# MohammadJohari/myslam

Measured on AMD Instinct MI355X. Metric: ray.samples/s (render+bwd), higher is better.
Workload: dtype f32; 1 GPU; BASELINE configs[1]: Replica room0 (synthetic), 4096 rays x 64 samples (56+8); mapping iteration: sample + render fwd + loss + bwd (planes+decoders), no optimiser; rays_of_the_job=4096, rays_this_rank=4096, samples_per_ray=64, plane_bytes=27147008, planes_layout=channels_last, parallelism=single GPU, launch=hipGraph replay of the captured iteration

## Files before the change

myslam_amd/csrc/eslam_decode_tile.h:

```cpp
#pragma once
#include "eslam_common.h"

__device__ __forceinline__ int piece_channel(int g, int i) { return i < 4 ? 4 * g + i : 12 + 4 * g + i; }

template <bool CL>
__device__ __forceinline__ void gather8(const eslam_plane_t& P, float u, float v, int q, float acc[8]) {
    const AxisCoord ax = axis_coord(u, P.w);
    const AxisCoord ay = axis_coord(v, P.h);
    const float w00 = (1.0f - ax.t) * (1.0f - ay.t);
    const float w01 = ax.t * (1.0f - ay.t);
    const float w10 = (1.0f - ax.t) * ay.t;
    const float w11 = ax.t * ay.t;
    const unsigned sy = (unsigned)P.stride_y, sx = (unsigned)P.stride_x;
    const unsigned r0 = ay.i0 * sy, r1 = ay.i1 * sy;
    const unsigned c0 = ax.i0 * sx, c1 = ax.i1 * sx;
    const float* __restrict__ data = P.data;
    if (CL) {
        const unsigned q4 = 4u * q;
        const unsigned o00 = r0 + c0 + q4, o01 = r0 + c1 + q4, o10 = r1 + c0 + q4, o11 = r1 + c1 + q4;
        const float4_t a00 = *(const float4_t*)(data + o00), b00 = *(const float4_t*)(data + o00 + 16u);
        const float4_t a01 = *(const float4_t*)(data + o01), b01 = *(const float4_t*)(data + o01 + 16u);
        const float4_t a10 = *(const float4_t*)(data + o10), b10 = *(const float4_t*)(data + o10 + 16u);
        const float4_t a11 = *(const float4_t*)(data + o11), b11 = *(const float4_t*)(data + o11 + 16u);
#pragma unroll
        for (int i = 0; i < 4; ++i) {
            acc[i] += a00[i] * w00 + a01[i] * w01 + a10[i] * w10 + a11[i] * w11;
            acc[4 + i] += b00[i] * w00 + b01[i] * w01 + b10[i] * w10 + b11[i] * w11;
        }
    } else {
        const unsigned sc = (unsigned)P.stride_c;
#pragma unroll
        for (int i = 0; i < 8; ++i) {
            const unsigned co = (unsigned)piece_channel(q, i) * sc;
            acc[i] += data[co + r0 + c0] * w00 + data[co + r0 + c1] * w01 + data[co + r1 + c0] * w10 +
                      data[co + r1 + c1] * w11;
        }
    }
}

struct DecFrag {
    float w1[16];
    float4_t w2;
    float4_t w3;
    float4_t b1, b2;
    float4_t b3;
};

__device__ __forceinline__ void load_dec_frag(DecFrag& f, const float* L, int r, int q) {
#pragma unroll
    for (int lvl = 0; lvl < 2; ++lvl) {
        const float4_t a = *(const float4_t*)(L + DEC_W1 + r * 64 + lvl * 32 + 4 * q);
        const float4_t b = *(const float4_t*)(L + DEC_W1 + r * 64 + lvl * 32 + 16 + 4 * q);
#pragma unroll
        for (int i = 0; i < 4; ++i) {
            f.w1[lvl * 8 + i] = a[i];
            f.w1[lvl * 8 + 4 + i] = b[i];
        }
    }
    f.w2 = *(const float4_t*)(L + DEC_W2 + r * 16 + 4 * q);
    f.w3 = *(const float4_t*)(L + DEC_W3 + (r & 3) * 16 + 4 * q);
    f.b1 = *(const float4_t*)(L + DEC_B1 + 4 * q);
    f.b2 = *(const float4_t*)(L + DEC_B2 + 4 * q);
    f.b3 = *(const float4_t*)(L + DEC_B3);
}

__device__ __forceinline__ void mlp_hidden2(const DecFrag& f, const float4_t& h1, float4_t& h2) {
    float4_t a2 = f.b2;
#pragma unroll
    for (int ks = 0; ks < 4; ++ks) a2 = mfma16(f.w2[ks], h1[ks], a2);
#pragma unroll
    for (int i = 0; i < 4; ++i) h2[i] = fmaxf(a2[i], 0.0f);
}

__device__ __forceinline__ void mlp_hidden(const DecFrag& f, const float feat[16], float4_t& h1, float4_t& h2) {
    float4_t a1 = f.b1;
#pragma unroll
    for (int ks = 0; ks < 16; ++ks) a1 = mfma16(f.w1[ks], feat[ks], a1);
#pragma unroll
    for (int i = 0; i < 4; ++i) h1[i] = fmaxf(a1[i], 0.0f);
    mlp_hidden2(f, h1, h2);
}

__device__ __forceinline__ int64_t hidden_blocks(int S) { return (S + 15) >> 4; }

__device__ __forceinline__ void mlp_out_accum(const DecFrag& f, const float4_t& h2, int b, int r, float4_t& out) {
    const bool mine = (r >> 2) == b;
#pragma unroll
    for (int ks = 0; ks < 4; ++ks) out = mfma16(mine ? f.w3[ks] : 0.0f, h2[ks], out);
}

#define GATHER_PIPELINE 1

struct PlaneTaps {
    float4_t a00, b00, a01, b01, a10, b10, a11, b11;
    float w00, w01, w10, w11;
};

__device__ __forceinline__ void issue_taps(const eslam_plane_t& P, float u, float v, int q, PlaneTaps& t) {
    const AxisCoord ax = axis_coord(u, P.w);
    const AxisCoord ay = axis_coord(v, P.h);
    t.w00 = (1.0f - ax.t) * (1.0f - ay.t);
    t.w01 = ax.t * (1.0f - ay.t);
    t.w10 = (1.0f - ax.t) * ay.t;
    t.w11 = ax.t * ay.t;
    const unsigned sy = (unsigned)P.stride_y, sx = (unsigned)P.stride_x;
    const unsigned r0 = ay.i0 * sy, r1 = ay.i1 * sy;
    const unsigned c0 = ax.i0 * sx, c1 = ax.i1 * sx;
    const float* __restrict__ data = P.data;
    const unsigned q4 = 4u * q;
    const unsigned o00 = r0 + c0 + q4, o01 = r0 + c1 + q4, o10 = r1 + c0 + q4, o11 = r1 + c1 + q4;
    t.a00 = *(const float4_t*)(data + o00); t.b00 = *(const float4_t*)(data + o00 + 16u);
    t.a01 = *(const float4_t*)(data + o01); t.b01 = *(const float4_t*)(data + o01 + 16u);
    t.a10 = *(const float4_t*)(data + o10); t.b10 = *(const float4_t*)(data + o10 + 16u);
    t.a11 = *(const float4_t*)(data + o11); t.b11 = *(const float4_t*)(data + o11 + 16u);
}

__device__ __forceinline__ void accumulate_taps(const PlaneTaps& t, float acc[8]) {
#pragma unroll
    for (int i = 0; i < 4; ++i) {
        acc[i] += t.a00[i] * t.w00 + t.a01[i] * t.w01 + t.a10[i] * t.w10 + t.a11[i] * t.w11;
        acc[4 + i] += t.b00[i] * t.w00 + t.b01[i] * t.w01 + t.b10[i] * t.w10 + t.b11[i] * t.w11;
    }
}

template <bool CL>
__device__ __forceinline__ void gather_features(const PlaneSet& planes, int d, float x, float y, float z, int q,
                                                float feat[16], int opaque0) {
#pragma unroll
    for (int i = 0; i < 16; ++i) feat[i] = 0.0f;
    if (CL && GATHER_PIPELINE) {
        constexpr int D = GATHER_PIPELINE + 1;
        PlaneTaps taps[D];
// ... 250 lines not shown
```

myslam_amd/csrc/eslam_mlp_bwd_dev.h:

```cpp
#pragma once
#include <type_traits>
#include "eslam_decode_tile.h"
#include "eslam_loss_final.h"

struct RayUp { float gd, gr, gg, gb; };

__device__ __forceinline__ float4_t composite_bwd_chunk(const RayUp up, float beta, bool valid, float sd, float z, float cr,
                                                        float cg, float cb, float g_sdf_s, float trans_in, float& carry,
                                                        float& gbeta_acc, int lane) {
    const float sg = sigmoidf_(-sd * beta);
    const float e = expf(-beta * sg);
    const float alpha = valid ? 1.0f - e : 0.0f;
    const float fac = valid ? (1.0f - alpha) + 1e-10f : 1.0f;
    const float pin = wave_incl_prod(fac, lane);
    const float pex = wave_up1(pin, 1.0f);
    const float T = trans_in * pex;
    const float w = alpha * T;
    const float gw = (up.gd != 0.0f ? up.gd * z : 0.0f) + up.gr * cr + up.gg * cg + up.gb * cb;
    const float v = valid ? gw * w : 0.0f;
    const float vn = wave_down1(v, 0.0f);
    const float after_local = wave_incl_suffix_sum(vn, lane);
    const float after = after_local + carry;
    const float g_alpha = gw * T - after / fac;
    carry += wave_lane<0>(after_local) + wave_lane<0>(v);
// ... 13 lines not shown
}

#define TP 20
#define TPF 68
#define TPH 72

struct RayBwdIn {
    const float* z_vals;
    const float* sdf;
    const float* raw_rgb;
    const float* beta;
    const float* g_depth;
    const float* g_rgb;
    const float* g_sdf;
    float* beta_parts;
    int R, S;
};

struct MlpBwdArgs {
    eslam_decoders_t dec;
    const float* feat;
    const float* g_o;
    int64_t N;
    float* g_feat;
    float* slabs;
    RayBwdIn rb;
    LossGradIn li;
    const float* hid;
};

struct MlpBwdLane {
    int d;
    int lane, wave;
    int r, q;
    int gp, gq;
};

__device__ __forceinline__ MlpBwdLane mlp_bwd_lane() {
    MlpBwdLane ln;
    ln.d = blockIdx.y;
    ln.lane = threadIdx.x & 63; ln.wave = threadIdx.x >> 6;
    ln.r = ln.lane & 15; ln.q = ln.lane >> 4;
    ln.gp = ln.lane >> 2; ln.gq = ln.lane & 3;
    return ln;
}

template <class T> __device__ __forceinline__ void mlp_bwd_touch(const T x) { asm volatile("" :: "v"(x)); }

struct MlpBwdLdsAll {
    __attribute__((aligned(16))) float wlds[2 * DEC_LDS];
    __attribute__((aligned(16))) float gtile[4][64 * 4];
};
template <bool LOWP> struct MlpBwdLdsWgrad {
    __attribute__((aligned(16))) float tiles[4][4][16 * TP];
    __attribute__((aligned(16))) float ftile[4][LOWP ? 16 * TPH / 2 : 16 * TPF];
    __attribute__((aligned(16))) float comb[4][SLAB];
};
struct MlpBwdLdsRays { float beta_part[4]; };
template <int> struct MlpBwdLdsNone {};
template <int MODE, bool WGRAD, bool LOWP>
struct MlpBwdLds : MlpBwdLdsAll, std::conditional_t<WGRAD, MlpBwdLdsWgrad<LOWP>, MlpBwdLdsNone<0>>,
                   std::conditional_t<MODE != 0, MlpBwdLdsRays, MlpBwdLdsNone<1>> {};

template <bool GZ> struct MlpBwdFragF32 {
    DecFrag f;
    float w3col[4], w2t[4], w1t[4][4];

    __device__ __forceinline__ void load(const float* wlds, const MlpBwdLane& ln) {
        const float* L = wlds + ln.d * DEC_LDS;
        const int r = ln.r, q = ln.q;
        load_dec_frag(f, L, r, q);
#pragma unroll
        for (int ks = 0; ks < 4; ++ks) {
            w3col[ks] = L[DEC_W3 + ks * 16 + r];
            w2t[ks] = L[DEC_W2 + (4 * q + ks) * 16 + r];
#pragma unroll
            for (int mb = 0; mb < 4; ++mb)
                if (!GZ) w1t[mb][ks] = L[DEC_W1 + (4 * q + ks) * 64 + (mb >> 1) * 32 + 16 * (mb & 1) + r];
        }
    }
};

struct MlpBwdFragBf16 {
    DecFragLP fl;
    short4_t w3colp = {0, 0, 0, 0}, w2tp = {0, 0, 0, 0}, w1tp[4];

    __device__ __forceinline__ void load(float* wlds, const MlpBwdLane& ln) {
        const int r = ln.r, q = ln.q;
        const short* W = lp_weights(wlds, ln.d);
        load_dec_frag_lp(fl, W, lp_biases(wlds, ln.d), r, q);
#pragma unroll
        for (int jj = 0; jj < 4; ++jj) {
            if (q == 0) w3colp[jj] = W[LP_W3 + jj * 16 + r];
            w2tp[jj] = W[LP_W2 + (4 * q + jj) * 16 + r];
#pragma unroll
            for (int mb = 0; mb < 4; ++mb) w1tp[mb][jj] = W[LP_W1 + (4 * q + jj) * 64 + 16 * mb + r];
        }
    }
};

template <bool LOWP, bool GZ> using MlpBwdFrag = std::conditional_t<LOWP, MlpBwdFragBf16, MlpBwdFragF32<GZ>>;

struct MlpBwdParamGrads {
    float4_t gW1[4], gW2, gW3, gb1, gb2;
    float gb3[3];

    __device__ __forceinline__ void clear() {
#pragma unroll
        for (int i = 0; i < 4; ++i) gW1[i] = (float4_t){0.f, 0.f, 0.f, 0.f};
        gW2 = gW3 = gb1 = gb2 = (float4_t){0.f, 0.f, 0.f, 0.f};
        gb3[0] = gb3[1] = gb3[2] = 0.f;
    }

    __device__ __forceinline__ void write_slab(float (*comb)[SLAB], float* __restrict__ slabs, const MlpBwdLane& ln) const {
        const int lane = ln.lane, r = ln.r, q = ln.q;
        const int nout = ln.d ? 3 : 1;
        float* sl = comb[ln.wave];
        for (int i = lane; i < SLAB; i += WAVE) sl[i] = 0.0f;
        WAVE_SYNC();
#pragma unroll
        for (int reg = 0; reg < 4; ++reg) {
            const int j = 4 * q + reg;
            float4_t v;
#pragma unroll
            for (int nb = 0; nb < 4; ++nb) v[nb] = gW1[nb][reg];
            *(float4_t*)(sl + SL_W1 + j * 64 + 4 * r) = v;
            sl[SL_W2 + j * 16 + r] = gW2[reg];
            if (q == 0 && reg < nout) sl[SL_W3 + reg * 16 + r] = gW3[reg];
        }
#pragma unroll
        for (int reg = 0; reg < 4; ++reg) {
            float a = gb1[reg], c = gb2[reg];
#pragma unroll
            for (int m = 8; m >= 1; m >>= 1) {
                a += __shfl_xor(a, m, WAVE);
                c += __shfl_xor(c, m, WAVE);
            }
            if (r == 0) {
                sl[SL_B1 + 4 * q + reg] = a;
                sl[SL_B2 + 4 * q + reg] = c;
            }
        }
#pragma unroll
        for (int o = 0; o < 3; ++o) {
            const float t = wave_sum(gb3[o]);
            if (lane == 0 && o < nout) sl[SL_B3 + o] = t;
        }
        __syncthreads();
        float* row = slabs + ((int64_t)blockIdx.x * 2 + ln.d) * SLAB;
        for (int col = threadIdx.x; col < SLAB; col += 256)
            row[col] = (comb[0][col] + comb[1][col]) + (comb[2][col] + comb[3][col]);
    }
};

template <bool GZ> struct MlpBwdGradOut {
    typedef unsigned uint4_t __attribute__((ext_vector_type(4)));
    __amdgpu_buffer_rsrc_t rsrc;
    unsigned gz_base;
    int d, gp, gq;

    __device__ __forceinline__ MlpBwdGradOut(float* g_feat, int64_t N, const MlpBwdLane& ln)
        : rsrc(__builtin_amdgcn_make_buffer_rsrc((void*)g_feat, 0, (int)((unsigned)N * (GZ ? 128u : 512u)), 0x00020000)),
          gz_base((unsigned)ln.d * ((unsigned)N * 64u)), d(ln.d), gp(ln.gp), gq(ln.gq) {}

    __device__ __forceinline__ void dropped_stores() const {
#pragma unroll
        for (int j = 0; j < (GZ ? 1 : 4); ++j) __builtin_amdgcn_raw_buffer_store_b128((uint4_t){0u, 0u, 0u, 0u}, rsrc, (int)(0xFFFFFF00u + 16u * j), 0, 0);
    }
    __device__ __forceinline__ void store_gz(const int64_t p0, const int b, const int nvalid, const float gzr[4]) const {
        const unsigned off = (16 * b + gp < nvalid) ? (unsigned)(p0 + 16 * b + gp) * 64u + gz_base + (unsigned)(gq * 16) : 0xFFFFFF00u;
        __builtin_amdgcn_raw_buffer_store_b128(__builtin_bit_cast(uint4_t, (float4_t){gzr[0], gzr[1], gzr[2], gzr[3]}), rsrc, (int)off, 0, 0);
    }
    __device__ __forceinline__ void store_rows(const int64_t p0, const int b, const int nvalid, const float gf[16]) const {
        const unsigned off = (16 * b + gp < nvalid) ? (unsigned)(p0 + 16 * b + gp) * 512u + (unsigned)(d * 256 + gq * 16) : 0xFFFFFF00u;
#pragma unroll
        for (int j = 0; j < 4; ++j)
            __builtin_amdgcn_raw_buffer_store_b128(__builtin_bit_cast(uint4_t, (float4_t){gf[4 * j], gf[4 * j + 1], gf[4 * j + 2], gf[4 * j + 3]}),
                                                   rsrc, (int)off + 64 * j, 0, 0);
    }
};

template <bool LOWP, bool ROWS, bool SAVEDH> struct MlpBwdPrefetch {
    float4_t fnext[4];
    float4_t hnext = (float4_t){0.f, 0.f, 0.f, 0.f};

    static __device__ __forceinline__ void load_block(const MlpBwdArgs& a, const MlpBwdLane& ln, float4_t v[4], const int64_t pbase) {
        const int64_t pt = min(pbase + ln.gp, a.N - 1);
        if (LOWP) {
            const short* fp = (const short*)a.feat + pt * 128 + ln.d * 64 + 8 * ln.gq;
            v[0] = *(const float4_t*)(fp);
            v[1] = *(const float4_t*)(fp + 32);
            v[2] = v[3] = (float4_t){0.f, 0.f, 0.f, 0.f};
            return;
        }
        const float* fp = a.feat + pt * 128 + ln.d * 64 + 4 * ln.gq;
        v[0] = *(const float4_t*)(fp);
        v[1] = *(const float4_t*)(fp + 16);
        v[2] = *(const float4_t*)(fp + 32);
        v[3] = *(const float4_t*)(fp + 48);
    }
    static __device__ __forceinline__ float4_t load_hidden(const MlpBwdArgs& a, const MlpBwdLane& ln, const int64_t hblk) {
        const int64_t hb_last = 2 * (int64_t)a.rb.R * hidden_blocks(a.rb.S) - 1;
        return *(const float4_t*)(a.hid + min(hblk, hb_last) * 256 + ln.lane * 4);
    }
    __device__ __forceinline__ void request(const MlpBwdArgs& a, const MlpBwdLane& ln, const int64_t pbase, const int64_t hblk) {
        if (ROWS) load_block(a, ln, fnext, pbase);
        if (SAVEDH) hnext = load_hidden(a, ln, hblk);
    }
    __device__ __forceinline__ void touch() const {
        if (ROWS) { mlp_bwd_touch(fnext[0]); mlp_bwd_touch(fnext[1]); mlp_bwd_touch(fnext[2]); mlp_bwd_touch(fnext[3]); }
        if (SAVEDH) mlp_bwd_touch(hnext);
    }
};

struct MlpBwdBlockOut { float4_t h1, h2, gz1, gz2; };

struct MlpBwdContract { float az1[4], az2[4], bh1[4], bh2[4], ago[4]; };
template <class Lds>
__device__ __forceinline__ MlpBwdContract mlp_bwd_transpose(Lds& lds, const MlpBwdLane& ln, const int b, const MlpBwdBlockOut& o) {
    const int r = ln.r, q = ln.q;
    float* tz1 = lds.tiles[ln.wave][0];
    float* tz2 = lds.tiles[ln.wave][1];
    float* th1 = lds.tiles[ln.wave][2];
    float* th2 = lds.tiles[ln.wave][3];
    const float* gt = lds.gtile[ln.wave];
    *(float4_t*)(tz1 + r * TP + 4 * q) = o.gz1;
    *(float4_t*)(tz2 + r * TP + 4 * q) = o.gz2;
    *(float4_t*)(th1 + r * TP + 4 * q) = o.h1;
    *(float4_t*)(th2 + r * TP + 4 * q) = o.h2;
    WAVE_SYNC();

    MlpBwdContract c;
#pragma unroll
    for (int ks = 0; ks < 4; ++ks) {
        const int prow = 4 * q + ks;
        c.az1[ks] = tz1[prow * TP + r];
        c.az2[ks] = tz2[prow * TP + r];
        c.bh1[ks] = th1[prow * TP + r];
        c.bh2[ks] = th2[prow * TP + r];
        c.ago[ks] = (r < 4) ? gt[(16 * b + prow) * 4 + r] : 0.0f;
    }
    return c;
}

__device__ __forceinline__ void mlp_bwd_stage_rows_f32(float* ftile, const MlpBwdLane& ln, const float ft[16]) {
    float* T = ftile + ln.gp * TPF + 4 * ln.gq;
#pragma unroll
    for (int j = 0; j < 4; ++j) *(float4_t*)(T + 16 * j) = (float4_t){ft[4 * j], ft[4 * j + 1], ft[4 * j + 2], ft[4 * j + 3]};
}

template <bool SAVEDH>
__device__ __forceinline__ void mlp_bwd_hidden_f32(const DecFrag& f, const float ft[16], const float4_t hsaved, float4_t& h1, float4_t& h2) {
    if (SAVEDH) { h1 = hsaved; mlp_hidden2(f, h1, h2); }
    else mlp_hidden(f, ft, h1, h2);
}

template <bool GZ>
__device__ __forceinline__ void mlp_bwd_w3_w2_f32(const MlpBwdFragF32<GZ>& w, const int q, const int b, const float go[4],
                                                  MlpBwdParamGrads& pg, MlpBwdBlockOut& o) {
    float4_t gh2 = (float4_t){0.f, 0.f, 0.f, 0.f};
    const bool mine = (q == b);
#pragma unroll
    for (int ks = 0; ks < 4; ++ks) gh2 = mfma16(mine ? w.w3col[ks] : 0.0f, go[ks], gh2);
#pragma unroll
    for (int i = 0; i < 4; ++i) o.gz2[i] = o.h2[i] > 0.0f ? gh2[i] : 0.0f;
    float4_t gh1 = (float4_t){0.f, 0.f, 0.f, 0.f};
#pragma unroll
    for (int ks = 0; ks < 4; ++ks) gh1 = mfma16(w.w2t[ks], o.gz2[ks], gh1);
#pragma unroll
    for (int i = 0; i < 4; ++i) o.gz1[i] = o.h1[i] > 0.0f ? gh1[i] : 0.0f;
    pg.gb1 += o.gz1;
    pg.gb2 += o.gz2;
}

__device__ __forceinline__ void mlp_bwd_store_gz1(const MlpBwdGradOut<true>& out, const int lane, const int64_t p0, const int b,
                                                  const int nvalid, const float4_t gz1) {
    float gzr[4] = {gz1[0], gz1[1], gz1[2], gz1[3]};
    to_gather_role<true, 4>(gzr, lane);
    out.store_gz(p0, b, nvalid, gzr);
}

__device__ __forceinline__ void mlp_bwd_w1_rows_f32(const MlpBwdFragF32<false>& w, const MlpBwdGradOut<false>& out, const int lane,
                                                    const int64_t p0, const int b, const int nvalid, const float4_t gz1) {
    float gf[16];
#pragma unroll
    for (int mb = 0; mb < 4; ++mb) {
        float4_t acc = (float4_t){0.f, 0.f, 0.f, 0.f};
#pragma unroll
        for (int ks = 0; ks < 4; ++ks) acc = mfma16(w.w1t[mb][ks], gz1[ks], acc);
#pragma unroll
        for (int i = 0; i < 4; ++i) gf[(mb >> 1) * 8 + 4 * (mb & 1) + i] = acc[i];
    }
    to_gather_role<true, 16>(gf, lane);
    out.store_rows(p0, b, nvalid, gf);
}

template <class Lds>
__device__ __forceinline__ void mlp_bwd_wgrad_f32(Lds& lds, const MlpBwdLane& ln, const int b, const MlpBwdBlockOut& o,
                                                  MlpBwdParamGrads& pg) {
    const MlpBwdContract c = mlp_bwd_transpose(lds, ln, b, o);
    float4_t fbk[4];
#pragma unroll
    for (int ks = 0; ks < 4; ++ks) {
        pg.gW2 = mfma16(c.az2[ks], c.bh1[ks], pg.gW2);
        pg.gW3 = mfma16(c.ago[ks], c.bh2[ks], pg.gW3);
    }
#pragma unroll
    for (int ks = 0; ks < 4; ++ks) fbk[ks] = *(const float4_t*)(lds.ftile[ln.wave] + (4 * ln.q + ks) * TPF + 4 * ln.r);
#pragma unroll
    for (int ks = 0; ks < 4; ++ks) {
#pragma unroll
        for (int nb = 0; nb < 4; ++nb) pg.gW1[nb] = mfma16(c.az1[ks], fbk[ks][nb], pg.gW1[nb]);
    }
    WAVE_SYNC();
}

template <bool WGRAD, bool GZ, bool SAVEDH, class Lds>
__device__ __forceinline__ void mlp_bwd_block_f32(Lds& lds, const MlpBwdLane& ln, const MlpBwdFragF32<GZ>& w, MlpBwdParamGrads& pg,
                                                  const MlpBwdGradOut<GZ>& out, float ft[16], const float4_t hsaved, const float go[4],
                                                  const int64_t p0, const int b, const int nvalid) {
    if constexpr (WGRAD) mlp_bwd_stage_rows_f32(lds.ftile[ln.wave], ln, ft);
    if (!SAVEDH) to_mfma_role<true, 16>(ft, ln.lane);
    MlpBwdBlockOut o;
    mlp_bwd_hidden_f32<SAVEDH>(w.f, ft, hsaved, o.h1, o.h2);
    mlp_bwd_w3_w2_f32(w, ln.q, b, go, pg, o);
    if constexpr (GZ) mlp_bwd_store_gz1(out, ln.lane, p0, b, nvalid, o.gz1);
    else mlp_bwd_w1_rows_f32(w, out, ln.lane, p0, b, nvalid, o.gz1);
    if constexpr (WGRAD) mlp_bwd_wgrad_f32(lds, ln, b, o, pg);
}

__device__ __forceinline__ void mlp_bwd_stage_rows_bf16(float* ftile, const MlpBwdLane& ln, const float ft[16]) {
    short* T = (short*)ftile + ln.gp * TPH + 8 * ln.gq;
    *(float4_t*)(T) = (float4_t){ft[0], ft[1], ft[2], ft[3]};
    *(float4_t*)(T + 32) = (float4_t){ft[4], ft[5], ft[6], ft[7]};
}

__device__ __forceinline__ void mlp_bwd_hidden_bf16(const DecFragLP& fl, const float ft[16], float4_t& a1, float4_t& a2, float4_t& h1,
                                                    float4_t& h2) {
    short8_t bfeat[2];
#pragma unroll
    for (int lvl = 0; lvl < 2; ++lvl)
#pragma unroll
        for (int i = 0; i < 4; ++i) {
            const unsigned u = __builtin_bit_cast(unsigned, ft[lvl * 4 + i]);
            bfeat[lvl][2 * i] = (short)(u & 0xFFFFu);
            bfeat[lvl][2 * i + 1] = (short)(u >> 16);
        }
    mlp_hidden_lp_bf(fl, bfeat, a1, a2);
#pragma unroll
    for (int i = 0; i < 4; ++i) { h1[i] = fmaxf(a1[i], 0.f); h2[i] = fmaxf(a2[i], 0.f); }
}

__device__ __forceinline__ void mlp_bwd_w3_w2_bf16(const MlpBwdFragBf16& w, const MlpBwdLane& ln, const int b, const float go[4],
                                                   const float4_t a1, const float4_t a2, MlpBwdParamGrads& pg, MlpBwdBlockOut& o) {
    const int r = ln.r, q = ln.q;
    const float4_t zero4 = (float4_t){0.f, 0.f, 0.f, 0.f};
    const float s0 = __shfl(go[0], 16 * b + r, WAVE), s1 = __shfl(go[1], 16 * b + r, WAVE), s2 = __shfl(go[2], 16 * b + r, WAVE);
    const short4_t bgo = (q == 0) ? pack4(s0, s1, s2, 0.f) : (short4_t){0, 0, 0, 0};
    const float4_t gh2 = __builtin_amdgcn_mfma_f32_16x16x16bf16_1k(w.w3colp, bgo, zero4, 0, 0, 0);
#pragma unroll
    for (int i = 0; i < 4; ++i) o.gz2[i] = a2[i] > 0.0f ? gh2[i] : 0.0f;
    const float4_t gh1 = __builtin_amdgcn_mfma_f32_16x16x16bf16_1k(w.w2tp, pack4(o.gz2[0], o.gz2[1], o.gz2[2], o.gz2[3]), zero4, 0, 0, 0);
#pragma unroll
    for (int i = 0; i < 4; ++i) o.gz1[i] = a1[i] > 0.0f ? gh1[i] : 0.0f;
    pg.gb1 += o.gz1;
    pg.gb2 += o.gz2;
}

__device__ __forceinline__ void mlp_bwd_w1_rows_bf16(const MlpBwdFragBf16& w, const MlpBwdGradOut<false>& out, const int lane,
                                                     const int64_t p0, const int b, const int nvalid, const float4_t gz1) {
    const float4_t zero4 = (float4_t){0.f, 0.f, 0.f, 0.f};
    float gf[16];
    const short4_t bz1 = pack4(gz1[0], gz1[1], gz1[2], gz1[3]);
#pragma unroll
    for (int mb = 0; mb < 4; ++mb) {
        const float4_t acc = __builtin_amdgcn_mfma_f32_16x16x16bf16_1k(w.w1tp[mb], bz1, zero4, 0, 0, 0);
#pragma unroll
        for (int i = 0; i < 4; ++i) gf[4 * mb + i] = acc[i];
    }
    to_gather_role<true, 16>(gf, lane);
    out.store_rows(p0, b, nvalid, gf);
}

template <class Lds>
__device__ __forceinline__ void mlp_bwd_wgrad_bf16(Lds& lds, const MlpBwdLane& ln, const int b, const MlpBwdBlockOut& o,
                                                   MlpBwdParamGrads& pg) {
    const MlpBwdContract c = mlp_bwd_transpose(lds, ln, b, o);
    short4_t fbkp[4];
    pg.gW2 = __builtin_amdgcn_mfma_f32_16x16x16bf16_1k(pack4(c.az2[0], c.az2[1], c.az2[2], c.az2[3]),
                                                       pack4(c.bh1[0], c.bh1[1], c.bh1[2], c.bh1[3]), pg.gW2, 0, 0, 0);
    pg.gW3 = __builtin_amdgcn_mfma_f32_16x16x16bf16_1k(pack4(c.ago[0], c.ago[1], c.ago[2], c.ago[3]),
                                                       pack4(c.bh2[0], c.bh2[1], c.bh2[2], c.bh2[3]), pg.gW3, 0, 0, 0);
    const short4_t a1p = pack4(c.az1[0], c.az1[1], c.az1[2], c.az1[3]);
#pragma unroll
    for (int ks = 0; ks < 4; ++ks) fbkp[ks] = *(const short4_t*)((const short*)lds.ftile[ln.wave] + (4 * ln.q + ks) * TPH + 4 * ln.r);
#pragma unroll
    for (int nb = 0; nb < 4; ++nb)
        pg.gW1[nb] = __builtin_amdgcn_mfma_f32_16x16x16bf16_1k(a1p, (short4_t){fbkp[0][nb], fbkp[1][nb], fbkp[2][nb], fbkp[3][nb]},
                                                               pg.gW1[nb], 0, 0, 0);
    WAVE_SYNC();
}

template <bool WGRAD, class Lds>
__device__ __forceinline__ void mlp_bwd_block_bf16(Lds& lds, const MlpBwdLane& ln, const MlpBwdFragBf16& w, MlpBwdParamGrads& pg,
                                                   const MlpBwdGradOut<false>& out, float ft[16], const float go[4], const int64_t p0,
                                                   const int b, const int nvalid) {
    if constexpr (WGRAD) mlp_bwd_stage_rows_bf16(lds.ftile[ln.wave], ln, ft);
    to_mfma_role<true, 8>(ft, ln.lane);
    MlpBwdBlockOut o;
    float4_t a1, a2;
    mlp_bwd_hidden_bf16(w.fl, ft, a1, a2, o.h1, o.h2);
    mlp_bwd_w3_w2_bf16(w, ln, b, go, a1, a2, pg, o);
    mlp_bwd_w1_rows_bf16(w, out, ln.lane, p0, b, nvalid, o.gz1);
    if constexpr (WGRAD) mlp_bwd_wgrad_bf16(lds, ln, b, o, pg);
}

template <bool WGRAD, bool LOWP, bool GZ, bool SAVEDH, class Lds, class Prefetch>
__device__ __forceinline__ void mlp_bwd_tile(const MlpBwdArgs& a, Lds& lds, const MlpBwdLane& ln, const MlpBwdFrag<LOWP, GZ>& w, MlpBwdParamGrads& pg,
                                             const MlpBwdGradOut<GZ>& out, Prefetch& pf, const int64_t p0, const int nvalid,
                                             const float go[4], const int64_t p0_next, const int64_t hb, const int64_t hb_next) {
    constexpr bool ROWS = !SAVEDH || WGRAD;
    const int nblk = (nvalid + 15) >> 4;
    __builtin_assume(nblk >= 1);
#pragma unroll
    for (int o = 0; o < 3; ++o) pg.gb3[o] += go[o];
    *(float4_t*)(lds.gtile[ln.wave] + ln.lane * 4) = (float4_t){go[0], go[1], go[2], go[3]};

#pragma unroll 1
    for (int b = 0; b < nblk; ++b) {
        float ft[16];
        if (ROWS) {
            const float4_t f0 = pf.fnext[0], f1 = pf.fnext[1], f2 = pf.fnext[2], f3 = pf.fnext[3];
#pragma unroll
            for (int i = 0; i < 4; ++i) {
                ft[i] = f0[i]; ft[4 + i] = f1[i]; ft[8 + i] = f2[i]; ft[12 + i] = f3[i];
            }
        }
        const float4_t hsaved = pf.hnext;
        pf.request(a, ln, b + 1 < nblk ? p0 + 16 * (b + 1) : p0_next, b + 1 < nblk ? hb + b + 1 : hb_next);
        if constexpr (LOWP) mlp_bwd_block_bf16<WGRAD>(lds, ln, w, pg, out, ft, go, p0, b, nvalid);
        else mlp_bwd_block_f32<WGRAD, GZ, SAVEDH>(lds, ln, w, pg, out, ft, hsaved, go, p0, b, nvalid);
    }
}

template <bool WGRAD, bool LOWP, class Lds, class Prefetch>
__device__ __forceinline__ void mlp_bwd_points(const MlpBwdArgs& a, Lds& lds, const MlpBwdLane& ln, const MlpBwdFrag<LOWP, false>& w,
                                               MlpBwdParamGrads& pg, const MlpBwdGradOut<false>& out, Prefetch& pf) {
    const int64_t N = a.N;
    const int64_t ntiles = (N + 63) / 64;
    int64_t tile = (int64_t)blockIdx.x * 4 + ln.wave;
    if (tile < ntiles) {
        pf.request(a, ln, tile * 64, 0);
        out.dropped_stores();
    }
    for (; tile < ntiles; tile += (int64_t)gridDim.x * 4) {
        const int64_t p0 = tile * 64;
        const int nvalid = (int)min((int64_t)64, N - p0);
        float go[4] = {0.f, 0.f, 0.f, 0.f};
        if (ln.lane < nvalid) {
            const float4_t g = *(const float4_t*)(a.g_o + (p0 + ln.lane) * 4);
            if (ln.d == 0) go[0] = g[3];
            else { go[0] = g[0]; go[1] = g[1]; go[2] = g[2]; }
        }
        pf.touch();
        mlp_bwd_tile<WGRAD, LOWP, false, false>(a, lds, ln, w, pg, out, pf, p0, nvalid, go, (tile + (int64_t)gridDim.x * 4) * 64, 0, 0);
    }
}

struct RayIn {
    float gd, gr, gg, gb, gtd, dep, cr, cg, cb, tr, tg, tb;
    int mask;

    template <int MODE> static __device__ __forceinline__ RayIn load(const RayBwdIn& rb, const LossGradIn& li, int ray) {
        RayIn x;
        x.gd = rb.g_depth ? rb.g_depth[ray] : 0.0f;
        x.gr = rb.g_rgb ? rb.g_rgb[3 * ray + 0] : 0.0f;
        x.gg = rb.g_rgb ? rb.g_rgb[3 * ray + 1] : 0.0f;
        x.gb = rb.g_rgb ? rb.g_rgb[3 * ray + 2] : 0.0f;
        x.gtd = x.dep = x.cr = x.cg = x.cb = x.tr = x.tg = x.tb = 0.0f;
        x.mask = 1;
        if (MODE == 2) {
            x.gtd = li.gt_depth[ray];
            x.mask = li.ray_mask ? (int)li.ray_mask[ray] : 1;
            x.dep = li.depth[ray];
            x.cr = li.rgb[3 * ray + 0]; x.cg = li.rgb[3 * ray + 1]; x.cb = li.rgb[3 * ray + 2];
            x.tr = li.gt_color[3 * ray + 0]; x.tg = li.gt_color[3 * ray + 1]; x.tb = li.gt_color[3 * ray + 2];
        }
        return x;
    }
    __device__ __forceinline__ void touch() const {
        mlp_bwd_touch(gd); mlp_bwd_touch(gr); mlp_bwd_touch(gg); mlp_bwd_touch(gb); mlp_bwd_touch(gtd); mlp_bwd_touch(dep);
        mlp_bwd_touch(cr); mlp_bwd_touch(cg); mlp_bwd_touch(cb); mlp_bwd_touch(tr); mlp_bwd_touch(tg); mlp_bwd_touch(tb);
        mlp_bwd_touch(mask);
    }
};

struct ChunkIn {
    float sd, z, cr, cg, cb, gs;

    static __device__ __forceinline__ ChunkIn load(const RayBwdIn& rb, int ray, int c, int lane) {
// ... 26 lines not shown
        for (int k = 0; k < 3; ++k)
            if (k < nchunk - 1) x.sd[k] = rb.sdf[(int64_t)ray * rb.S + k * WAVE + lane];
        return x;
    }
    __device__ __forceinline__ void touch() const { mlp_bwd_touch(sd[0]); mlp_bwd_touch(sd[1]); mlp_bwd_touch(sd[2]); }
};

template <int MODE> struct RayLossGrad {
    LossW lw = {};
    LossK lk = {};
    float nd = 1.0f, ncol = 1.0f;

    __device__ __forceinline__ explicit RayLossGrad(const LossGradIn& li) {
        if (MODE == 2) {
            lw = loss_scaled_weights(li.w, li.upstream);
            lk = loss_sdf_factors(lw, li.tr, li.acc);
            nd = li.acc[A_N_DEPTH]; ncol = li.acc[A_N_COLOR];
            if (blockIdx.x == 0 && blockIdx.y == 0 && threadIdx.x == 0 && li.loss_out)
                li.loss_out[0] = loss_value_from_acc(li.w, li.acc);
        }
    }
    __device__ __forceinline__ void upstream(const RayIn& rin, RayUp& up, bool& m) const {
        up.gd = rin.gd; up.gr = rin.gr; up.gg = rin.gg; up.gb = rin.gb;
        m = false;
        if (MODE == 2) {
            const bool mc = rin.mask != 0;
            m = mc && rin.gtd > 0.0f;
            up.gd += loss_g_depth(m, rin.gtd, rin.dep, lw, nd);
            up.gr += loss_g_color(mc, rin.tr, rin.cr, lw, ncol);
            up.gg += loss_g_color(mc, rin.tg, rin.cg, lw, ncol);
            up.gb += loss_g_color(mc, rin.tb, rin.cb, lw, ncol);
        }
    }
};

__device__ __forceinline__ float ray_pass_a(const PassA& pin, const float beta, const int nchunk, const int lane) {
    float myprod = 1.0f;
#pragma unroll
    for (int c = 0; c < 3; ++c) {
        if (c < nchunk - 1) {
            const float sd = pin.sd[c];
            const float alpha = 1.0f - expf(-beta * sigmoidf_(-sd * beta));
            const float cp = wave_lane<63>(wave_incl_prod((1.0f - alpha) + 1e-10f, lane));
            if (lane == c) myprod = cp;
        }
    }
    return myprod;
}

__device__ __forceinline__ int64_t ray_hidden_block(int d, int R, int64_t SB, int ray, int c) { return ((int64_t)d * R + ray) * SB + 4 * c; }

template <int MODE, bool WGRAD, bool LOWP, bool GZ, bool SAVEDH, class Lds, class Prefetch>
__device__ __forceinline__ float mlp_bwd_rays(const MlpBwdArgs& a, Lds& lds, const MlpBwdLane& ln, const MlpBwdFrag<LOWP, GZ>& w,
                                              MlpBwdParamGrads& pg, const MlpBwdGradOut<GZ>& out, Prefetch& pf) {
    const RayBwdIn& rb = a.rb;
    const LossGradIn& li = a.li;
    const int lane = ln.lane, d = ln.d;
    const int R = rb.R, S = rb.S;
    const int nchunk = (S + WAVE - 1) / WAVE;
    const int64_t SB = hidden_blocks(S);
    __builtin_assume(nchunk >= 1);
    const float beta = rb.beta[0];
    const RayLossGrad<MODE> loss(li);
    float gbeta_acc = 0.0f;
    const int stride = gridDim.x * 4;
    int ray = blockIdx.x * 4 + ln.wave;
    RayIn rin = {};
    ChunkIn cin = {};
    PassA pin = {{0.f, 0.f, 0.f}};
    if (ray < R) {
        rin = RayIn::load<MODE>(rb, li, ray);
        cin = ChunkIn::load(rb, ray, nchunk - 1, lane);
        pin = PassA::load(rb, ray, nchunk, lane);
        pf.request(a, ln, (int64_t)ray * S + (nchunk - 1) * WAVE, ray_hidden_block(d, R, SB, ray, nchunk - 1));
    }
    out.dropped_stores();
    for (; ray < R; ray += stride) {
        const int64_t base = (int64_t)ray * S;
        rin.touch();
        cin.touch();
        pin.touch();
        pf.touch();
        ChunkIn ch = cin;
        RayIn rnx = {};
        ChunkIn cnx = {};
        PassA pnx = {{0.f, 0.f, 0.f}};
        if (ray + stride < R) {
            rnx = RayIn::load<MODE>(rb, li, ray + stride);
            cnx = ChunkIn::load(rb, ray + stride, nchunk - 1, lane);
            pnx = PassA::load(rb, ray + stride, nchunk, lane);
        }
        RayUp up;
        bool m;
        loss.upstream(rin, up, m);
        const float gtd = rin.gtd;
        const float myprod = ray_pass_a(pin, beta, nchunk, lane);
        float carry = 0.0f;
        int c = nchunk - 1;
        do {
            ChunkIn cn = {};
            if (c > 0) cn = ChunkIn::load(rb, ray, c - 1, lane);
            float trans_in = 1.0f;
            for (int k = 0; k < c; ++k) trans_in *= __shfl(myprod, k, WAVE);
            const bool valid = c * WAVE + lane < S;
            float gs = ch.gs;
            if (MODE == 2 && valid) gs += loss_g_sdf(m, ch.z, ch.sd, gtd, li.tr, loss.lk);
            const float4_t o = composite_bwd_chunk(up, beta, valid, ch.sd, ch.z, ch.cr, ch.cg, ch.cb, gs, trans_in, carry,
// ... 29 lines not shown
```

myslam_amd/csrc/eslam_render_bwd.hip:

```cpp
#include <stdlib.h>
#include "eslam_decode_tile.h"
#include "eslam_loss_final.h"
#include "eslam_dec_reduce.h"
#include "eslam_mlp_bwd_dev.h"

__global__ void decode_act_bwd_kernel(const float* __restrict__ raw, const float* __restrict__ g_raw, int64_t N,
                                      float* __restrict__ g_o) {
    const int64_t i = (int64_t)blockIdx.x * blockDim.x + threadIdx.x;
    if (i >= N) return;
    const float4_t v = *(const float4_t*)(raw + 4 * i);
    const float4_t g = *(const float4_t*)(g_raw + 4 * i);
    float4_t o;
    o[0] = g[0] * v[0] * (1.0f - v[0]);
    o[1] = g[1] * v[1] * (1.0f - v[1]);
    o[2] = g[2] * v[2] * (1.0f - v[2]);
    o[3] = g[3] * (1.0f - v[3] * v[3]);
    *(float4_t*)(g_o + 4 * i) = o;
}

template <int MODE, bool WGRAD, bool LOWP, bool GZ = false, bool SAVEDH = false>
__global__ __launch_bounds__(256, 2) void mlp_bwd_kernel(const MlpBwdArgs a) {
    static_assert(!GZ || (!LOWP && MODE != 0), "GZ: float32 rays only");
    static_assert(!SAVEDH || (!LOWP && MODE != 0), "SAVEDH: float32 rays only");
    constexpr bool ROWS = !SAVEDH || WGRAD;
    __shared__ MlpBwdLds<MODE, WGRAD, LOWP> lds;
    if (LOWP) stage_decoder_weights_lowp(lds.wlds, a.dec, threadIdx.x, blockDim.x);
    else stage_decoder_weights(lds.wlds, a.dec, threadIdx.x, blockDim.x);
    __syncthreads();

    const MlpBwdLane ln = mlp_bwd_lane();
    MlpBwdFrag<LOWP, GZ> w;
    w.load(lds.wlds, ln);
    MlpBwdParamGrads pg;
    pg.clear();
    const MlpBwdGradOut<GZ> out(a.g_feat, a.N, ln);
    MlpBwdPrefetch<LOWP, ROWS, SAVEDH> pf;

    if constexpr (MODE == 0) {
        mlp_bwd_points<WGRAD, LOWP>(a, lds, ln, w, pg, out, pf);
    } else {
        const float gbeta_acc = mlp_bwd_rays<MODE, WGRAD, LOWP, GZ, SAVEDH>(a, lds, ln, w, pg, out, pf);
        mlp_bwd_beta_partial(lds.beta_part, a.rb.beta_parts, gbeta_acc, ln);
    }
    if constexpr (WGRAD) pg.write_slab(lds.comb, a.slabs, ln);
}

__global__ __launch_bounds__(1024) void beta_sum_kernel(const float* __restrict__ parts, int n, float* __restrict__ out) {
    __shared__ float bsum[16];
    float a = 0.f;
    for (int i = threadIdx.x; i < n; i += 1024) a += parts[i];
    a = wave_sum(a);
    if ((threadIdx.x & 63) == 0) bsum[threadIdx.x >> 6] = a;
    __syncthreads();
    if (threadIdx.x == 0) {
        float t = 0.f;
        for (int k = 0; k < 16; ++k) t += bsum[k];
        out[0] = t;
    }
}

__global__ __launch_bounds__(1024) void dec_grad_reduce_kernel(const DecReduceArgs a) {
    __shared__ float red[16 * 64];
    dec_grad_reduce_block<1024>(a, blockIdx.x, blockIdx.y, red);
}

template <bool CL>
__device__ __forceinline__ void coord_grad8(const eslam_plane_t& P, float u, float v, int q, const float g[8],
                                            float& gu, float& gv) {
    const AxisCoord ax = axis_coord(u, P.w);
    const AxisCoord ay = axis_coord(v, P.h);
    const int sy = (int)P.stride_y, sx = (int)P.stride_x, sc = (int)P.stride_c;
    const int r0 = ay.i0 * sy, r1 = ay.i1 * sy, c0 = ax.i0 * sx, c1 = ax.i1 * sx;
    float su = 0.f, sv = 0.f;
    if (CL) {
        const float* base = P.data + 4 * q;
#pragma unroll
        for (int hh = 0; hh < 2; ++hh) {
            const float4_t t00 = *(const float4_t*)(base + r0 + c0 + 16 * hh);
            const float4_t t01 = *(const float4_t*)(base + r0 + c1 + 16 * hh);
            const float4_t t10 = *(const float4_t*)(base + r1 + c0 + 16 * hh);
            const float4_t t11 = *(const float4_t*)(base + r1 + c1 + 16 * hh);
#pragma unroll
            for (int i = 0; i < 4; ++i) {
                su += g[4 * hh + i] * ((t01[i] - t00[i]) * (1.0f - ay.t) + (t11[i] - t10[i]) * ay.t);
                sv += g[4 * hh + i] * ((t10[i] - t00[i]) * (1.0f - ax.t) + (t11[i] - t01[i]) * ax.t);
            }
// ... 519 lines not shown
```

Measured before the change: 1.281 billion ray.samples/s.

## Compute W3 backward with lane FMAs instead of sparse MFMAs in f32 path

```diff
diff --git a/myslam_amd/csrc/eslam_decode_tile.h b/myslam_amd/csrc/eslam_decode_tile.h
--- a/myslam_amd/csrc/eslam_decode_tile.h
+++ b/myslam_amd/csrc/eslam_decode_tile.h
@@ -72,12 +72,15 @@
     for (int i = 0; i < 4; ++i) h2[i] = fmaxf(a2[i], 0.0f);
 }
 
+__device__ __forceinline__ void mlp_hidden1(const DecFrag& f, const float feat[16], float4_t& h1) {
+    float4_t a1 = f.b1;
+#pragma unroll
+    for (int ks = 0; ks < 16; ++ks) a1 = mfma16(f.w1[ks], feat[ks], a1);
+#pragma unroll
+    for (int i = 0; i < 4; ++i) h1[i] = fmaxf(a1[i], 0.0f);
+}
 __device__ __forceinline__ void mlp_hidden(const DecFrag& f, const float feat[16], float4_t& h1, float4_t& h2) {
-    float4_t a1 = f.b1;
-#pragma unroll
-    for (int ks = 0; ks < 16; ++ks) a1 = mfma16(f.w1[ks], feat[ks], a1);
-#pragma unroll
-    for (int i = 0; i < 4; ++i) h1[i] = fmaxf(a1[i], 0.0f);
+    mlp_hidden1(f, feat, h1);
     mlp_hidden2(f, h1, h2);
 }
 
diff --git a/myslam_amd/csrc/eslam_mlp_bwd_dev.h b/myslam_amd/csrc/eslam_mlp_bwd_dev.h
--- a/myslam_amd/csrc/eslam_mlp_bwd_dev.h
+++ b/myslam_amd/csrc/eslam_mlp_bwd_dev.h
@@ -89,7 +89,7 @@
     __attribute__((aligned(16))) float gtile[4][64 * 4];
 };
 template <bool LOWP> struct MlpBwdLdsWgrad {
-    __attribute__((aligned(16))) float tiles[4][4][16 * TP];
+    __attribute__((aligned(16))) float tiles[4][LOWP ? 4 : 3][16 * TP];
     __attribute__((aligned(16))) float ftile[4][LOWP ? 16 * TPH / 2 : 16 * TPF];
     __attribute__((aligned(16))) float comb[4][SLAB];
 };
@@ -101,7 +101,7 @@
 
 template <bool GZ> struct MlpBwdFragF32 {
     DecFrag f;
-    float w3col[4], w2t[4], w1t[4][4];
+    float w2t[4], w1t[4][4];
 
     __device__ __forceinline__ void load(const float* wlds, const MlpBwdLane& ln) {
         const float* L = wlds + ln.d * DEC_LDS;
@@ -109,7 +109,6 @@
         load_dec_frag(f, L, r, q);
 #pragma unroll
         for (int ks = 0; ks < 4; ++ks) {
-            w3col[ks] = L[DEC_W3 + ks * 16 + r];
             w2t[ks] = L[DEC_W2 + (4 * q + ks) * 16 + r];
 #pragma unroll
             for (int mb = 0; mb < 4; ++mb)
@@ -138,15 +137,33 @@
 
 template <bool LOWP, bool GZ> using MlpBwdFrag = std::conditional_t<LOWP, MlpBwdFragBf16, MlpBwdFragF32<GZ>>;
 
-struct MlpBwdParamGrads {
-    float4_t gW1[4], gW2, gW3, gb1, gb2;
+struct MlpBwdGradW3Mfma { float4_t gW3; };
+struct MlpBwdGradW3Lane { float4_t w3_0, w3_1, w3_2; };
+
+template <bool LOWP> struct MlpBwdParamGrads : std::conditional_t<LOWP, MlpBwdGradW3Mfma, MlpBwdGradW3Lane> {
+    float4_t gW1[4], gW2, gb1, gb2;
     float gb3[3];
 
     __device__ __forceinline__ void clear() {
 #pragma unroll
         for (int i = 0; i < 4; ++i) gW1[i] = (float4_t){0.f, 0.f, 0.f, 0.f};
-        gW2 = gW3 = gb1 = gb2 = (float4_t){0.f, 0.f, 0.f, 0.f};
+        gW2 = gb1 = gb2 = (float4_t){0.f, 0.f, 0.f, 0.f};
+        if constexpr (LOWP) this->gW3 = (float4_t){0.f, 0.f, 0.f, 0.f};
+        else this->w3_0 = this->w3_1 = this->w3_2 = (float4_t){0.f, 0.f, 0.f, 0.f};
         gb3[0] = gb3[1] = gb3[2] = 0.f;
+    }
+
+    static __device__ __forceinline__ void store_w3_row(float* sl_row, float4_t v, const int r, const int q, const bool wanted) {
+#pragma unroll
+        for (int i = 0; i < 4; ++i) {
+            float t = v[i];
+            t += dpp_from<0x111, 0xf>(0.0f, t);
+            t += dpp_from<0x112, 0xf>(0.0f, t);
+            t += dpp_from<0x114, 0xf>(0.0f, t);
+            t += dpp_from<0x118, 0xf>(0.0f, t);
+            v[i] = t;
+        }
+        if (r == 15 && wanted) *(float4_t*)(sl_row + 4 * q) = v;
     }
 
     __device__ __forceinline__ void write_slab(float (*comb)[SLAB], float* __restrict__ slabs, const MlpBwdLane& ln) const {
@@ -163,7 +180,14 @@
             for (int nb = 0; nb < 4; ++nb) v[nb] = gW1[nb][reg];
             *(float4_t*)(sl + SL_W1 + j * 64 + 4 * r) = v;
             sl[SL_W2 + j * 16 + r] = gW2[reg];
-            if (q == 0 && reg < nout) sl[SL_W3 + reg * 16 + r] = gW3[reg];
+            if constexpr (LOWP) {
+                if (q == 0 && reg < nout) sl[SL_W3 + reg * 16 + r] = this->gW3[reg];
+            }
+        }
+        if constexpr (!LOWP) {
+            store_w3_row(sl + SL_W3, this->w3_0, r, q, true);
+            store_w3_row(sl + SL_W3 + 16, this->w3_1, r, q, nout == 3);
+            store_w3_row(sl + SL_W3 + 32, this->w3_2, r, q, nout == 3);
         }
 #pragma unroll
         for (int reg = 0; reg < 4; ++reg) {
@@ -252,30 +276,31 @@
 
 struct MlpBwdBlockOut { float4_t h1, h2, gz1, gz2; };
 
-struct MlpBwdContract { float az1[4], az2[4], bh1[4], bh2[4], ago[4]; };
-template <class Lds>
-__device__ __forceinline__ MlpBwdContract mlp_bwd_transpose(Lds& lds, const MlpBwdLane& ln, const int b, const MlpBwdBlockOut& o) {
+struct MlpBwdContractW3 { float bh2[4], ago[4]; };
+template <bool LOWP> struct MlpBwdContract : std::conditional_t<LOWP, MlpBwdContractW3, MlpBwdLdsNone<2>> { float az1[4], az2[4], bh1[4]; };
+template <bool LOWP, class Lds>
+__device__ __forceinline__ MlpBwdContract<LOWP> mlp_bwd_transpose(Lds& lds, const MlpBwdLane& ln, const int b, const MlpBwdBlockOut& o) {
     const int r = ln.r, q = ln.q;
     float* tz1 = lds.tiles[ln.wave][0];
     float* tz2 = lds.tiles[ln.wave][1];
     float* th1 = lds.tiles[ln.wave][2];
-    float* th2 = lds.tiles[ln.wave][3];
-    const float* gt = lds.gtile[ln.wave];
     *(float4_t*)(tz1 + r * TP + 4 * q) = o.gz1;
     *(float4_t*)(tz2 + r * TP + 4 * q) = o.gz2;
     *(float4_t*)(th1 + r * TP + 4 * q) = o.h1;
-    *(float4_t*)(th2 + r * TP + 4 * q) = o.h2;
+    if constexpr (LOWP) *(float4_t*)(lds.tiles[ln.wave][3] + r * TP + 4 * q) = o.h2;
     WAVE_SYNC();
 
-    MlpBwdContract c;
+    MlpBwdContract<LOWP> c;
 #pragma unroll
     for (int ks = 0; ks < 4; ++ks) {
         const int prow = 4 * q + ks;
         c.az1[ks] = tz1[prow * TP + r];
         c.az2[ks] = tz2[prow * TP + r];
         c.bh1[ks] = th1[prow * TP + r];
-        c.bh2[ks] = th2[prow * TP + r];
-        c.ago[ks] = (r < 4) ? gt[(16 * b + prow) * 4 + r] : 0.0f;
+        if constexpr (LOWP) {
+            c.bh2[ks] = lds.tiles[ln.wave][3][prow * TP + r];
+            c.ago[ks] = (r < 4) ? lds.gtile[ln.wave][(16 * b + prow) * 4 + r] : 0.0f;
+        }
     }
     return c;
 }
@@ -287,18 +312,42 @@
 }
 
 template <bool SAVEDH>
-__device__ __forceinline__ void mlp_bwd_hidden_f32(const DecFrag& f, const float ft[16], const float4_t hsaved, float4_t& h1, float4_t& h2) {
-    if (SAVEDH) { h1 = hsaved; mlp_hidden2(f, h1, h2); }
-    else mlp_hidden(f, ft, h1, h2);
+__device__ __forceinline__ void mlp_bwd_hidden1_f32(const DecFrag& f, const float ft[16], const float4_t hsaved, float4_t& h1) {
+    if (SAVEDH) h1 = hsaved;
+    else mlp_hidden1(f, ft, h1);
+}
+
+struct MlpBwdOutIn {
+    float4_t g, w0, w1, w2;
+    template <class Lds> static __device__ __forceinline__ MlpBwdOutIn load(const Lds& lds, const MlpBwdLane& ln, const int b) {
+        const float* W3 = lds.wlds + ln.d * DEC_LDS + DEC_W3 + 4 * ln.q;
+        MlpBwdOutIn x;
+        x.g = *(const float4_t*)(lds.gtile[ln.wave] + (16 * b + ln.r) * 4);
+        x.w0 = *(const float4_t*)(W3);
+        x.w1 = *(const float4_t*)(W3 + 16);
+        x.w2 = *(const float4_t*)(W3 + 32);
+        return x;
+    }
+};
+template <bool WGRAD>
+__device__ __forceinline__ float4_t mlp_bwd_out_grads_f32(const MlpBwdOutIn& x, const float4_t h2, MlpBwdParamGrads<false>& pg) {
+    float4_t gh2;
+#pragma unroll
+    for (int i = 0; i < 4; ++i) gh2[i] = fmaf(x.w2[i], x.g[2], fmaf(x.w1[i], x.g[1], fmaf(x.w0[i], x.g[0], 0.0f)));
+    if constexpr (WGRAD) {
+#pragma unroll
+        for (int i = 0; i < 4; ++i) {
+            pg.w3_0[i] = fmaf(x.g[0], h2[i], pg.w3_0[i]);
+            pg.w3_1[i] = fmaf(x.g[1], h2[i], pg.w3_1[i]);
+            pg.w3_2[i] = fmaf(x.g[2], h2[i], pg.w3_2[i]);
+        }
+    }
+    return gh2;
 }
 
 template <bool GZ>
-__device__ __forceinline__ void mlp_bwd_w3_w2_f32(const MlpBwdFragF32<GZ>& w, const int q, const int b, const float go[4],
-                                                  MlpBwdParamGrads& pg, MlpBwdBlockOut& o) {
-    float4_t gh2 = (float4_t){0.f, 0.f, 0.f, 0.f};
-    const bool mine = (q == b);
-#pragma unroll
-    for (int ks = 0; ks < 4; ++ks) gh2 = mfma16(mine ? w.w3col[ks] : 0.0f, go[ks], gh2);
+__device__ __forceinline__ void mlp_bwd_w3_w2_f32(const MlpBwdFragF32<GZ>& w, const float4_t gh2, MlpBwdParamGrads<false>& pg,
+                                                  MlpBwdBlockOut& o) {
 #pragma unroll
     for (int i = 0; i < 4; ++i) o.gz2[i] = o.h2[i] > 0.0f ? gh2[i] : 0.0f;
     float4_t gh1 = (float4_t){0.f, 0.f, 0.f, 0.f};
@@ -334,18 +383,15 @@
 
 template <class Lds>
 __device__ __forceinline__ void mlp_bwd_wgrad_f32(Lds& lds, const MlpBwdLane& ln, const int b, const MlpBwdBlockOut& o,
-                                                  MlpBwdParamGrads& pg) {
-    const MlpBwdContract c = mlp_bwd_transpose(lds, ln, b, o);
+                                                  MlpBwdParamGrads<false>& pg) {
+    const MlpBwdContract<false> c = mlp_bwd_transpose<false>(lds, ln, b, o);
     float4_t fbk[4];
 #pragma unroll
+    for (int ks = 0; ks < 4; ++ks) pg.gW2 = mfma16(c.az2[ks], c.bh1[ks], pg.gW2);
+#pragma unroll
+    for (int ks = 0; ks < 4; ++ks) fbk[ks] = *(const float4_t*)(lds.ftile[ln.wave] + (4 * ln.q + ks) * TPF + 4 * ln.r);
+#pragma unroll
     for (int ks = 0; ks < 4; ++ks) {
-        pg.gW2 = mfma16(c.az2[ks], c.bh1[ks], pg.gW2);
-        pg.gW3 = mfma16(c.ago[ks], c.bh2[ks], pg.gW3);
-    }
-#pragma unroll
-    for (int ks = 0; ks < 4; ++ks) fbk[ks] = *(const float4_t*)(lds.ftile[ln.wave] + (4 * ln.q + ks) * TPF + 4 * ln.r);
-#pragma unroll
-    for (int ks = 0; ks < 4; ++ks) {
 #pragma unroll
         for (int nb = 0; nb < 4; ++nb) pg.gW1[nb] = mfma16(c.az1[ks], fbk[ks][nb], pg.gW1[nb]);
     }
@@ -353,14 +399,17 @@
 }
 
 template <bool WGRAD, bool GZ, bool SAVEDH, class Lds>
-__device__ __forceinline__ void mlp_bwd_block_f32(Lds& lds, const MlpBwdLane& ln, const MlpBwdFragF32<GZ>& w, MlpBwdParamGrads& pg,
-                                                  const MlpBwdGradOut<GZ>& out, float ft[16], const float4_t hsaved, const float go[4],
+__device__ __forceinline__ void mlp_bwd_block_f32(Lds& lds, const MlpBwdLane& ln, const MlpBwdFragF32<GZ>& w, MlpBwdParamGrads<false>& pg,
+                                                  const MlpBwdGradOut<GZ>& out, float ft[16], const float4_t hsaved,
                                                   const int64_t p0, const int b, const int nvalid) {
     if constexpr (WGRAD) mlp_bwd_stage_rows_f32(lds.ftile[ln.wave], ln, ft);
     if (!SAVEDH) to_mfma_role<true, 16>(ft, ln.lane);
     MlpBwdBlockOut o;
-    mlp_bwd_hidden_f32<SAVEDH>(w.f, ft, hsaved, o.h1, o.h2);
-    mlp_bwd_w3_w2_f32(w, ln.q, b, go, pg, o);
+    mlp_bwd_hidden1_f32<SAVEDH>(w.f, ft, hsaved, o.h1);
+    if constexpr (!SAVEDH) __builtin_amdgcn_sched_barrier(0);
+    const MlpBwdOutIn oi = MlpBwdOutIn::load(lds, ln, b);
+    mlp_hidden2(w.f, o.h1, o.h2);
+    mlp_bwd_w3_w2_f32(w, mlp_bwd_out_grads_f32<WGRAD>(oi, o.h2, pg), pg, o);
     if constexpr (GZ) mlp_bwd_store_gz1(out, ln.lane, p0, b, nvalid, o.gz1);
     else mlp_bwd_w1_rows_f32(w, out, ln.lane, p0, b, nvalid, o.gz1);
     if constexpr (WGRAD) mlp_bwd_wgrad_f32(lds, ln, b, o, pg);
@@ -389,7 +438,7 @@
 }
 
 __device__ __forceinline__ void mlp_bwd_w3_w2_bf16(const MlpBwdFragBf16& w, const MlpBwdLane& ln, const int b, const float go[4],
-                                                   const float4_t a1, const float4_t a2, MlpBwdParamGrads& pg, MlpBwdBlockOut& o) {
+                                                   const float4_t a1, const float4_t a2, MlpBwdParamGrads<true>& pg, MlpBwdBlockOut& o) {
     const int r = ln.r, q = ln.q;
     const float4_t zero4 = (float4_t){0.f, 0.f, 0.f, 0.f};
     const float s0 = __shfl(go[0], 16 * b + r, WAVE), s1 = __shfl(go[1], 16 * b + r, WAVE), s2 = __shfl(go[2], 16 * b + r, WAVE);
@@ -421,8 +470,8 @@
 
 template <class Lds>
 __device__ __forceinline__ void mlp_bwd_wgrad_bf16(Lds& lds, const MlpBwdLane& ln, const int b, const MlpBwdBlockOut& o,
-                                                   MlpBwdParamGrads& pg) {
-    const MlpBwdContract c = mlp_bwd_transpose(lds, ln, b, o);
+                                                   MlpBwdParamGrads<true>& pg) {
+    const MlpBwdContract<true> c = mlp_bwd_transpose<true>(lds, ln, b, o);
     short4_t fbkp[4];
     pg.gW2 = __builtin_amdgcn_mfma_f32_16x16x16bf16_1k(pack4(c.az2[0], c.az2[1], c.az2[2], c.az2[3]),
                                                        pack4(c.bh1[0], c.bh1[1], c.bh1[2], c.bh1[3]), pg.gW2, 0, 0, 0);
@@ -439,7 +488,7 @@
 }
 
 template <bool WGRAD, class Lds>
-__device__ __forceinline__ void mlp_bwd_block_bf16(Lds& lds, const MlpBwdLane& ln, const MlpBwdFragBf16& w, MlpBwdParamGrads& pg,
+__device__ __forceinline__ void mlp_bwd_block_bf16(Lds& lds, const MlpBwdLane& ln, const MlpBwdFragBf16& w, MlpBwdParamGrads<true>& pg,
                                                    const MlpBwdGradOut<false>& out, float ft[16], const float go[4], const int64_t p0,
                                                    const int b, const int nvalid) {
     if constexpr (WGRAD) mlp_bwd_stage_rows_bf16(lds.ftile[ln.wave], ln, ft);
@@ -453,7 +502,7 @@
 }
 
 template <bool WGRAD, bool LOWP, bool GZ, bool SAVEDH, class Lds, class Prefetch>
-__device__ __forceinline__ void mlp_bwd_tile(const MlpBwdArgs& a, Lds& lds, const MlpBwdLane& ln, const MlpBwdFrag<LOWP, GZ>& w, MlpBwdParamGrads& pg,
+__device__ __forceinline__ void mlp_bwd_tile(const MlpBwdArgs& a, Lds& lds, const MlpBwdLane& ln, const MlpBwdFrag<LOWP, GZ>& w, MlpBwdParamGrads<LOWP>& pg,
                                              const MlpBwdGradOut<GZ>& out, Prefetch& pf, const int64_t p0, const int nvalid,
                                              const float go[4], const int64_t p0_next, const int64_t hb, const int64_t hb_next) {
     constexpr bool ROWS = !SAVEDH || WGRAD;
@@ -461,7 +510,9 @@
     __builtin_assume(nblk >= 1);
 #pragma unroll
     for (int o = 0; o < 3; ++o) pg.gb3[o] += go[o];
+    if constexpr (!LOWP) WAVE_SYNC();
     *(float4_t*)(lds.gtile[ln.wave] + ln.lane * 4) = (float4_t){go[0], go[1], go[2], go[3]};
+    if constexpr (!LOWP) WAVE_SYNC();
 
 #pragma unroll 1
     for (int b = 0; b < nblk; ++b) {
@@ -476,13 +527,13 @@
         const float4_t hsaved = pf.hnext;
         pf.request(a, ln, b + 1 < nblk ? p0 + 16 * (b + 1) : p0_next, b + 1 < nblk ? hb + b + 1 : hb_next);
         if constexpr (LOWP) mlp_bwd_block_bf16<WGRAD>(lds, ln, w, pg, out, ft, go, p0, b, nvalid);
-        else mlp_bwd_block_f32<WGRAD, GZ, SAVEDH>(lds, ln, w, pg, out, ft, hsaved, go, p0, b, nvalid);
+        else mlp_bwd_block_f32<WGRAD, GZ, SAVEDH>(lds, ln, w, pg, out, ft, hsaved, p0, b, nvalid);
     }
 }
 
 template <bool WGRAD, bool LOWP, class Lds, class Prefetch>
 __device__ __forceinline__ void mlp_bwd_points(const MlpBwdArgs& a, Lds& lds, const MlpBwdLane& ln, const MlpBwdFrag<LOWP, false>& w,
-                                               MlpBwdParamGrads& pg, const MlpBwdGradOut<false>& out, Prefetch& pf) {
+                                               MlpBwdParamGrads<LOWP>& pg, const MlpBwdGradOut<false>& out, Prefetch& pf) {
     const int64_t N = a.N;
     const int64_t ntiles = (N + 63) / 64;
     int64_t tile = (int64_t)blockIdx.x * 4 + ln.wave;
@@ -615,7 +666,7 @@
 
 template <int MODE, bool WGRAD, bool LOWP, bool GZ, bool SAVEDH, class Lds, class Prefetch>
 __device__ __forceinline__ float mlp_bwd_rays(const MlpBwdArgs& a, Lds& lds, const MlpBwdLane& ln, const MlpBwdFrag<LOWP, GZ>& w,
-                                              MlpBwdParamGrads& pg, const MlpBwdGradOut<GZ>& out, Prefetch& pf) {
+                                              MlpBwdParamGrads<LOWP>& pg, const MlpBwdGradOut<GZ>& out, Prefetch& pf) {
     const RayBwdIn& rb = a.rb;
     const LossGradIn& li = a.li;
     const int lane = ln.lane, d = ln.d;
diff --git a/myslam_amd/csrc/eslam_render_bwd.hip b/myslam_amd/csrc/eslam_render_bwd.hip
--- a/myslam_amd/csrc/eslam_render_bwd.hip
+++ b/myslam_amd/csrc/eslam_render_bwd.hip
@@ -31,7 +31,7 @@
     const MlpBwdLane ln = mlp_bwd_lane();
     MlpBwdFrag<LOWP, GZ> w;
     w.load(lds.wlds, ln);
-    MlpBwdParamGrads pg;
+    MlpBwdParamGrads<LOWP> pg;
     pg.clear();
     const MlpBwdGradOut<GZ> out(a.g_feat, a.N, ln);
     MlpBwdPrefetch<LOWP, ROWS, SAVEDH> pf;
```

After: 1.287 billion ray.samples/s, median of 2. No clear change (+0.4%).
